# ChaitIITB/ReplicatingGPT

Hardware: AMD Instinct MI355X
Metric: train tokens/sec at 1/2/4/8 MI355X + MFMA util, char-GPT block 256 (higher is better)
Workload: dtype bf16; 1 GPU; c2: char-GPT 6L/6H/384d, block 256, batch 64/GPU, dropout 0.2, AdamW, full train step; global_batch=64, seq_len=256, parallelism=dp1, world_size=1, graph=True

## Files before the change

### include/charpt.h

```cpp
#ifndef CHARPT_H
#define CHARPT_H
#include <stdint.h>

#ifdef __cplusplus
extern "C" {
#endif

enum { CG_OK = 0, CG_EINVAL = 1, CG_EHIP = 2, CG_EUNSUPPORTED = 3 };
enum { CG_F32 = 0, CG_BF16 = 1 };
enum { CG_BITS = 2 };

enum {
    CG_EPI_STORE = 0,
    CG_EPI_BIAS = 1,
    CG_EPI_BIAS_RELU = 2,
    CG_EPI_BIAS_RESID = 3,
    CG_EPI_BIAS_DROP_RESID = 4,
    CG_EPI_RELU_BWD = 5,
    CG_EPI_STORE_ROWDOT = 7
};

typedef struct {
    int kind;
    const float* bias;
    const float* resid;
    int64_t ld_resid;
    const void* aux;
    int aux_dtype;
    int64_t ld_aux;
    double dropout_p;
    uint64_t seed;
    const uint64_t* rng_call;
    int site;
    float beta;
    float* colpart;
    int flags;
} cg_epilogue_t;

enum { CG_GEMM_SLAB_BF16 = 1, CG_GEMM_DEFER_REDUCE = 2 };
enum { CG_DEFER = 1 };

const char* cg_last_error_string(void);
int cg_version(void);
int cg_set_tuning(const char* key, int value);
int64_t cg_gemm_ws_launches(void);
int cg_device_info(int* n_cu, int* arch_major, int* arch_minor);
int cg_timing_event_create(void** event);
int cg_timing_event_record(void* event, void* stream);
int cg_timing_event_elapsed(void* start, void* end, float* ms);
int cg_timing_event_destroy(void* event);

int cg_counter_add(int64_t* counter, int64_t delta, void* stream);
int cg_rng_snapshot(uint64_t* counter, uint64_t* snap, void* stream);
int cg_dropout_mask(float* dst, int64_t n, double p, uint64_t seed, const uint64_t* rng_call, int site,
                    void* stream);
int cg_dropout_apply(const float* x, int64_t rows, int64_t C, int64_t ldx, void* y, int y_dtype, double p,
                     uint64_t seed, const uint64_t* rng_call, int site, void* stream);
int cg_sum_f32(const float* x, int64_t n, float scale, float* out, float* ws, void* stream);
int cg_cast_f32_bf16(const float* x, uint16_t* y, int64_t n, void* stream);

int cg_gather_batch(const void* data, int data_is_u8, const int64_t* ix, int64_t* x, int64_t* y,
                    int64_t B, int64_t T, void* stream);

int cg_gather_pairs(const int64_t* table, const int64_t* plen, const int64_t* tlen, const int64_t* ix, int64_t* x,
                    int64_t* y, int64_t B, int64_t T, int64_t pad_token, int64_t ignore_index, void* stream);

int cg_embed_fwd(const int64_t* idx, const float* wte, const float* wpe, float* x, int64_t B, int64_t T,
                 int64_t C, int64_t V, void* stream);
int64_t cg_embed_bwd_workspace(int64_t B, int64_t T, int64_t C, int64_t V);
int cg_embed_bwd(const int64_t* idx, const float* dx, float* dwte, float* dwpe, int64_t B, int64_t T,
                 int64_t C, int64_t V, int accumulate, void* workspace, void* stream);

int cg_layernorm_fwd(const float* x, const float* w, const float* b, void* y, int y_dtype, float* mean,
                     float* rstd, int64_t rows, int64_t C, float eps, void* stream);
int64_t cg_layernorm_bwd_workspace(int64_t rows, int64_t C);
int cg_layernorm_bwd(const void* dy, int dy_dtype, const float* x, const float* w, const float* mean,
                     const float* rstd, const float* dres, float* dx, uint16_t* dx_bf16, float* dw, float* db,
                     int accumulate, void* workspace, int64_t rows, int64_t C, void* stream);
int cg_layernorm_bwd_ex(const void* dy, int dy_dtype, const float* x, const float* w, const float* mean,
                        const float* rstd, const float* dres, float* dx, uint16_t* lp_out, double lp_dropout_p,
                        uint64_t lp_seed, const uint64_t* lp_rng_call, int lp_site, float* dw, float* db,
                        float* lp_colsum, int accumulate, int colsum_accumulate, void* workspace, int64_t rows,
                        int64_t C, void* stream);
int cg_layernorm_bwd_rows(const void* dy, int dy_dtype, const float* x, const float* w, const float* mean,
                          const float* rstd, const float* dres, float* dx, uint16_t* lp_out, double lp_dropout_p,
                          uint64_t lp_seed, const uint64_t* lp_rng_call, int lp_site, int lp_colsum,
                          void* workspace, int64_t rows, int64_t C, void* stream);
int cg_layernorm_bwd_reduce(const void* workspace, int64_t rows, int64_t C, int lp_colsum_partials, float* dw,
                            float* db, float* lp_colsum, int accumulate, int colsum_accumulate, void* stream);
int cg_layernorm_bwd_reduce_ex(const void* workspace, int64_t rows, int64_t C, int lp_colsum_partials, float* dw,
                               float* db, float* lp_colsum, int accumulate, int colsum_accumulate, int flags,
                               void* stream);

int64_t cg_gemm_workspace(int64_t M, int64_t N, int split_k);
int cg_gemm_colpart_supported(int a_trans, int b_trans, int64_t M, int64_t N, int64_t K, int64_t lda, int64_t ldb,
                              int64_t ldc);
int cg_gemm_relu_bits_supported(int a_trans, int b_trans, int64_t M, int64_t N, int64_t K, int64_t lda, int64_t ldb,
                                int64_t ldc);
// ... 145 lines not shown
```

### replicatinggpt_amd/_lib.py

```python
import ctypes
import os
import re

import torch

_HERE = os.path.dirname(os.path.abspath(__file__))
LIB_PATH = os.environ.get("CHARPT_LIB") or os.path.join(_HERE, "libcharpt_hip.so")
HEADER_PATH = os.path.join(os.path.dirname(_HERE), "include", "charpt.h")

CG_F32, CG_BF16, CG_BITS = 0, 1, 2
EPI_STORE, EPI_BIAS, EPI_BIAS_RELU, EPI_BIAS_RESID, EPI_BIAS_DROP_RESID, EPI_RELU_BWD = range(6)
EPI_STORE_ROWDOT = 7
GEMM_SLAB_BF16, GEMM_DEFER_REDUCE = 1, 2
DEFER = 1

c_i64, c_int, c_dbl, c_flt, c_u64, P = ctypes.c_int64, ctypes.c_int, ctypes.c_double, ctypes.c_float, ctypes.c_uint64, ctypes.c_void_p


class Epilogue(ctypes.Structure):
    _fields_ = [("kind", c_int), ("bias", P), ("resid", P), ("ld_resid", c_i64), ("aux", P), ("aux_dtype", c_int),
                ("ld_aux", c_i64), ("dropout_p", c_dbl), ("seed", c_u64), ("rng_call", P), ("site", c_int),
                ("beta", c_flt), ("colpart", P), ("flags", c_int)]


class WgradProblem(ctypes.Structure):
    _fields_ = [("M", c_i64), ("N", c_i64), ("K", c_i64), ("A", P), ("lda", c_i64), ("B", P), ("ldb", c_i64), ("C", P),
                ("ldc", c_i64), ("beta", c_flt), ("split_k", c_int), ("workspace", P), ("flags", c_int)]


_SIGS = {
    "cg_last_error_string": (ctypes.c_char_p, []),
    "cg_version": (c_int, []),
    "cg_set_tuning": (c_int, [ctypes.c_char_p, c_int]),
    "cg_device_info": (c_int, [P, P, P]),
    "cg_counter_add": (c_int, [P, c_i64, P]),
    "cg_rng_snapshot": (c_int, [P, P, P]),
    "cg_dropout_mask": (c_int, [P, c_i64, c_dbl, c_u64, P, c_int, P]),
    "cg_dropout_apply": (c_int, [P, c_i64, c_i64, c_i64, P, c_int, c_dbl, c_u64, P, c_int, P]),
    "cg_sum_f32": (c_int, [P, c_i64, c_flt, P, P, P]),
    "cg_cast_f32_bf16": (c_int, [P, P, c_i64, P]),
    "cg_gather_batch": (c_int, [P, c_int, P, P, P, c_i64, c_i64, P]),
    "cg_gather_pairs": (c_int, [P, P, P, P, P, P, c_i64, c_i64, c_i64, c_i64, P]),
    "cg_embed_fwd": (c_int, [P, P, P, P, c_i64, c_i64, c_i64, c_i64, P]),
    "cg_embed_bwd_workspace": (c_i64, [c_i64, c_i64, c_i64, c_i64]),
    "cg_embed_bwd": (c_int, [P, P, P, P, c_i64, c_i64, c_i64, c_i64, c_int, P, P]),
    "cg_layernorm_fwd": (c_int, [P, P, P, P, c_int, P, P, c_i64, c_i64, c_flt, P]),
    "cg_layernorm_bwd_workspace": (c_i64, [c_i64, c_i64]),
    "cg_layernorm_bwd": (c_int, [P, c_int, P, P, P, P, P, P, P, P, P, c_int, P, c_i64, c_i64, P]),
    "cg_layernorm_bwd_ex": (c_int, [P, c_int, P, P, P, P, P, P, P, c_dbl, c_u64, P, c_int, P, P, P, c_int, c_int, P,
                                    c_i64, c_i64, P]),
    "cg_layernorm_bwd_rows": (c_int, [P, c_int, P, P, P, P, P, P, P, c_dbl, c_u64, P, c_int, c_int, P, c_i64, c_i64,
                                      P]),
    "cg_layernorm_bwd_reduce": (c_int, [P, c_i64, c_i64, c_int, P, P, P, c_int, c_int, P]),
    "cg_layernorm_bwd_reduce_ex": (c_int, [P, c_i64, c_i64, c_int, P, P, P, c_int, c_int, c_int, P]),
    "cg_gemm_workspace": (c_i64, [c_i64, c_i64, c_int]),
    "cg_gemm_colpart_supported": (c_int, [c_int, c_int, c_i64, c_i64, c_i64, c_i64, c_i64, c_i64]),
    "cg_gemm_relu_bits_supported": (c_int, [c_int, c_int, c_i64, c_i64, c_i64, c_i64, c_i64, c_i64]),
    "cg_gemm_ws_launches": (c_i64, []),
    "cg_gemm_rowdot_supported": (c_int, [c_int, c_int, c_i64, c_i64, c_i64, c_i64, c_i64, c_i64]),
    "cg_linear_rows_f32_supported": (c_int, [c_i64, c_i64, c_i64]),
    "cg_decode_qkv_f32": (c_int, [c_i64, c_i64, c_i64, P, c_i64, P, P, c_flt, P, c_i64, P, c_i64, P, c_i64, P, P, P]),
    "cg_linear_rows_f32": (c_int, [c_i64, c_i64, c_i64, P, c_i64, P, P, c_flt, P, c_i64, P, c_int, P, c_i64, P, c_i64, P]),
    "cg_ffn_fwd_f32_supported": (c_int, [c_i64, c_i64, c_i64]),
    "cg_ffn_fwd_f32": (c_int, [c_i64, c_i64, c_i64, P, c_i64, P, P, c_flt, P, c_i64, P, P, c_i64, P, P, c_i64, P,
                               c_i64, P]),
    "cg_gemm_resid_layernorm_supported": (c_int, [c_i64, c_i64, c_i64]),
    "cg_gemm_resid_layernorm": (c_int, [c_i64, c_i64, c_i64, P, c_i64, P, c_i64, P, c_i64, ctypes.POINTER(Epilogue), P, P,
                                        P, P, P, c_flt, P]),
    "cg_flush_deferred": (c_int, [P]),
    "cg_discard_deferred": (c_int, [P, P]),
    "cg_reduce_rows": (c_int, [P, c_i64, c_i64, P, c_int, P]),
    "cg_reduce_rows_ex": (c_int, [P, c_i64, c_i64, P, c_int, c_int, P]),
    "cg_gemm": (c_int, [c_int, c_int, c_int, c_i64, c_i64, c_i64, P, c_i64, P, c_i64, P, c_int, c_i64,
                        ctypes.POINTER(Epilogue), c_int, P, P]),
    "cg_gemm_wgrad_group_supported": (c_int, [ctypes.POINTER(WgradProblem), c_int]),
    "cg_gemm_wgrad_group": (c_int, [ctypes.POINTER(WgradProblem), c_int, P]),
    "cg_colsum_workspace": (c_i64, [c_i64, c_i64]),
    "cg_colsum": (c_int, [P, c_int, c_i64, c_i64, c_i64, P, c_int, P, P]),
    "cg_attn_fwd": (c_int, [c_int, c_i64, c_i64, c_i64, c_i64, P, P, P, c_i64, P, c_i64, P, c_flt, c_dbl, c_u64, P,
                            c_int, P, P]),
    "cg_attn_fwd_premasked": (c_int, [c_int, c_i64, c_i64, c_i64, c_i64, P, P, P, c_i64, P, c_i64, P, c_flt, c_dbl,
                                      c_u64, P, c_int, P, P]),
    "cg_attn_dropmask": (c_int, [c_i64, c_i64, c_i64, c_dbl, c_u64, P, c_int, P, P]),
    "cg_layernorm_fwd_attn_dropmask": (c_int, [P, P, P, P, c_int, P, P, c_i64, c_i64, c_flt, c_i64, c_i64, c_i64,
                                               c_dbl, c_u64, P, c_int, P, P]),
    "cg_attn_mask_bytes": (c_i64, [c_i64, c_i64, c_i64]),
    "cg_attn_bwd_workspace": (c_i64, [c_i64, c_i64, c_i64, c_i64]),
    "cg_attn_bwd": (c_int, [c_int, c_i64, c_i64, c_i64, c_i64, P, P, P, c_i64, P, c_i64, P, c_i64, P, P, P, P, c_i64,
                            c_flt, c_dbl, c_u64, P, c_int, P, P, P]),
    "cg_attn_bwd_delta": (c_int, [c_int, c_i64, c_i64, c_i64, c_i64, P, P, P, c_i64, P, c_i64, P, c_i64, P, P, P, P,
                                  P, c_i64, c_flt, c_dbl, c_u64, P, c_int, P, P, P]),
    "cg_ce_fwd": (c_int, [P, c_i64, c_i64, c_i64, P, P, P, P]),
    "cg_ce_bwd": (c_int, [P, c_i64, c_i64, c_i64, P, P, P, c_flt, P, c_i64, P, P]),
    "cg_head_workspace": (c_i64, [c_i64, c_i64]),
    "cg_head_fwd": (c_int, [P, P, c_i64, P, P, P, P, P, P, c_i64, c_i64, c_i64, P]),
    "cg_head_bwd": (c_int, [P, P, P, P, c_flt, P, P, c_i64, P, c_int, P, c_i64, c_i64, P]),
    "cg_head_bwd_ex": (c_int, [P, P, P, P, c_flt, P, P, c_i64, P, c_int, P, c_i64, c_i64, c_int, P]),
    "cg_head_masked_workspace": (c_i64, [c_i64, c_i64]),
    "cg_head_fwd_masked": (c_int, [P, P, c_i64, P, P, c_i64, P, P, P, P, P, c_i64, c_i64, c_i64, P]),
    "cg_head_bwd_masked": (c_int, [P, P, P, c_i64, P, P, P, P, c_i64, P, c_int, P, c_i64, c_i64, c_int, P]),
    "cg_ce_fwd_masked": (c_int, [P, c_i64, c_i64, P, c_i64, P, P, P]),
    "cg_ce_mean_masked_workspace": (c_i64, [c_i64]),
    "cg_ce_mean_masked": (c_int, [P, P, c_i64, c_i64, P, P, P, P]),
    "cg_ce_bwd_masked": (c_int, [P, c_i64, c_i64, P, c_i64, P, P, P, P, P, P]),
    "cg_decode_window": (c_int, [P, c_i64, c_i64, c_i64, P, P, P]),
    "cg_decode_embed": (c_int, [P, c_i64, P, P, c_i64, P, P, c_i64, P]),
    "cg_decode_kv_append": (c_int, [P, c_i64, c_i64, c_i64, c_i64, c_i64, c_i64, c_i64, P, P, P, P]),
    "cg_decode_attn": (c_int, [P, c_i64, P, P, c_i64, c_i64, c_i64, c_i64, c_i64, c_i64, P, c_i64, c_flt, P, c_i64,
                               P]),
    "cg_decode_sample": (c_int, [P, c_i64, c_i64, c_i64, c_int, P, P, P, c_i64, P]),
    "cg_decode_sample_filtered": (c_int, [P, c_i64, c_i64, c_i64, P, P, P, P, c_i64, P]),
# ... 71 lines not shown
```

### replicatinggpt_amd/csrc/gemm.hip

```cpp
#include "defer.h"

using namespace cg;

namespace {

constexpr int GBM = 64, GBN = 64, GBK = 16;

template <typename TA, typename TB, typename TC>
__global__ __launch_bounds__(256) void k_gemm_generic(int a_trans, int b_trans, int64_t M, int64_t N, int64_t K,
                                                      const TA* __restrict__ A, int64_t lda,
                                                      const TB* __restrict__ B, int64_t ldb, TC* __restrict__ C,
                                                      int64_t ldc, EpiArgs epi, int split_k, int64_t kchunk,
                                                      float* __restrict__ ws) {
    __shared__ float As[GBK][GBM + 4];
    __shared__ float Bs[GBK][GBN + 4];
    const int tid = threadIdx.x, lane = tid & 63, wave = tid >> 6;
    const int wm = wave >> 1, wn = wave & 1;
    const int64_t tilesN = (N + GBN - 1) / GBN;
    const int64_t m0 = (int64_t)(blockIdx.x / tilesN) * GBM;
    const int64_t n0 = (int64_t)(blockIdx.x % tilesN) * GBN;
    const int split = blockIdx.y;
    const int64_t kb = split * kchunk;
    const int64_t ke = kb + kchunk < K ? kb + kchunk : K;

// ... 80 lines not shown
    a.aux_dtype = e->aux_dtype;
    a.ld_aux = e->ld_aux;
    a.thr = e->dropout_p > 0 ? dropout_threshold(e->dropout_p) : 0u;
    a.dscale = e->dropout_p > 0 ? dropout_scale(e->dropout_p) : 1.f;
    a.seed = e->seed;
    a.rng_call = e->rng_call;
    a.site = e->site;
    a.beta = e->beta;
    a.colpart = e->colpart;
    return a;
}

template <typename TA, typename TB>
int launch_generic(int a_trans, int b_trans, int64_t M, int64_t N, int64_t K, const void* A, int64_t lda,
                   const void* B, int64_t ldb, void* C, int c_dtype, int64_t ldc, const EpiArgs& e, int split_k,
                   void* ws, hipStream_t st) {
    int64_t kchunk = (K + split_k - 1) / split_k;
    kchunk = (kchunk + GBK - 1) / GBK * GBK;
    const int64_t tiles = ((M + GBM - 1) / GBM) * ((N + GBN - 1) / GBN);
    dim3 grid((unsigned)tiles, (unsigned)split_k);
    if (c_dtype == CG_BF16)
        k_gemm_generic<TA, TB, bf16_t><<<grid, 256, 0, st>>>(a_trans, b_trans, M, N, K, (const TA*)A, lda,
                                                             (const TB*)B, ldb, (bf16_t*)C, ldc, e, split_k, kchunk,
                                                             (float*)ws);
    else
        k_gemm_generic<TA, TB, float><<<grid, 256, 0, st>>>(a_trans, b_trans, M, N, K, (const TA*)A, lda,
                                                            (const TB*)B, ldb, (float*)C, ldc, e, split_k, kchunk,
                                                            (float*)ws);
    return CG_OK;
}

}

namespace cg {
int g_gemm_variant = 0;
int g_gemm_max_grid = 0;
int g_gemm_group_p8 = 0;
int g_gemm_group_pk = 0;
int g_gemm_n96 = 1;
}

extern "C" int cg_gemm_colpart_supported(int a_trans, int b_trans, int64_t M, int64_t N, int64_t K, int64_t lda,
                                         int64_t ldb, int64_t ldc) {
    return gemm_colpart_supported(a_trans, b_trans, M, N, K, lda, ldb, ldc) ? 1 : 0;
}

extern "C" int cg_gemm_relu_bits_supported(int a_trans, int b_trans, int64_t M, int64_t N, int64_t K, int64_t lda,
                                           int64_t ldb, int64_t ldc) {
    return gemm_relu_bits_supported(a_trans, b_trans, M, N, K, lda, ldb, ldc) ? 1 : 0;
}

extern "C" int64_t cg_gemm_ws_launches(void) { return (int64_t)ws_gemm_launches(); }

extern "C" int cg_gemm_rowdot_supported(int a_trans, int b_trans, int64_t M, int64_t N, int64_t K, int64_t lda,
                                        int64_t ldb, int64_t ldc) {
    return gemm_rowdot_supported(a_trans, b_trans, M, N, K, lda, ldb, ldc) ? 1 : 0;
}

extern "C" int64_t cg_gemm_workspace(int64_t M, int64_t N, int split_k) {
    return split_k > 1 ? (int64_t)split_k * M * N * (int64_t)sizeof(float) : 0;
}

extern "C" int cg_gemm_resid_layernorm_supported(int64_t M, int64_t N, int64_t K) {
    return gemm_resid_ln_supported(M, N, K) ? 1 : 0;
}

extern "C" int cg_gemm_resid_layernorm(int64_t M, int64_t N, int64_t K, const void* A, int64_t lda, const void* W,
                                       int64_t ldw, float* out, int64_t ldc, const cg_epilogue_t* epi,
                                       const float* ln_w, const float* ln_b, void* y, float* mean, float* rstd,
                                       float eps, void* stream) {
    CG_REQUIRE(gemm_resid_ln_supported(M, N, K),
               "cg_gemm_resid_layernorm: unsupported shape M=%lld N=%lld K=%lld (N == 384, M %% 64 == 0, K %% 64 == 0)",
               (long long)M, (long long)N, (long long)K);
    CG_REQUIRE(epi && (epi->kind == CG_EPI_BIAS_RESID || epi->kind == CG_EPI_BIAS_DROP_RESID) && epi->bias &&
                   epi->resid && epi->beta == 0.f && epi->flags == 0 && !epi->colpart,
               "cg_gemm_resid_layernorm: needs a BIAS_RESID / BIAS_DROP_RESID epilogue with bias and residual, beta 0");
    CG_REQUIRE(A && W && out && ln_w && ln_b && y && mean && rstd, "cg_gemm_resid_layernorm: null pointer");
    CG_REQUIRE(lda >= K && ldw >= K && lda % 8 == 0 && ldw % 8 == 0 && ldc >= N && ldc % 4 == 0 &&
                   epi->ld_resid >= N && epi->ld_resid % 4 == 0,
               "cg_gemm_resid_layernorm: bad leading dimensions");
    CG_REQUIRE((((uintptr_t)A | (uintptr_t)W | (uintptr_t)out | (uintptr_t)epi->resid | (uintptr_t)epi->bias |
                 (uintptr_t)ln_w | (uintptr_t)ln_b | (uintptr_t)y) & 15) == 0,
               "cg_gemm_resid_layernorm: operands must be 16-B aligned");
    const EpiArgs e = make_epi(epi);
    gemm_resid_ln_launch(M, K, (const bf16_t*)A, lda, (const bf16_t*)W, ldw, out, ldc, e, ln_w, ln_b, (bf16_t*)y, mean,
                         rstd, eps, (hipStream_t)stream);
    CG_LAUNCH_CHECK("cg_gemm_resid_layernorm");
    return CG_OK;
}

extern "C" int cg_gemm(int op_dtype, int a_trans, int b_trans, int64_t M, int64_t N, int64_t K, const void* A,
                       int64_t lda, const void* B, int64_t ldb, void* C, int c_dtype, int64_t ldc,
                       const cg_epilogue_t* epi, int split_k, void* workspace, void* stream) {
    CG_REQUIRE(M > 0 && N > 0 && K > 0, "cg_gemm: empty problem M=%lld N=%lld K=%lld", (long long)M, (long long)N,
               (long long)K);
    CG_REQUIRE(split_k >= 1 && split_k <= 64, "cg_gemm: split_k out of range");
    CG_REQUIRE(split_k == 1 || workspace, "cg_gemm: split_k > 1 needs a workspace");
    CG_REQUIRE(op_dtype == CG_BF16 || op_dtype == CG_F32, "cg_gemm: bad op dtype");
    hipStream_t st = (hipStream_t)stream;
    EpiArgs e = make_epi(epi);
    CG_REQUIRE(split_k == 1 || e.kind == CG_EPI_STORE || e.kind == CG_EPI_BIAS || e.kind == CG_EPI_BIAS_RESID,
               "cg_gemm: split-K supports STORE/BIAS/BIAS_RESID epilogues only");
    const bool vec4 = N % 4 == 0 && ldc % 4 == 0 && M * N < (int64_t)1 << 31 &&
                      (((uintptr_t)C | (uintptr_t)workspace | (uintptr_t)(e.bias ? e.bias : (const float*)C) |
                        (uintptr_t)(e.resid ? e.resid : (const float*)C)) & 15) == 0 &&
                      (!e.resid || e.ld_resid % 4 == 0);
// ... 131 lines not shown
```

### replicatinggpt_amd/csrc/gemm_common.h

```cpp
#pragma once
#include <type_traits>

#include "adamw.h"
#include "common.h"

namespace cg {

typedef float fv16f __attribute__((ext_vector_type(16)));

struct EpiArgs {
    int kind;
    const float* bias;
    const float* resid;
    int64_t ld_resid;
    const void* aux;
    int aux_dtype;
    int64_t ld_aux;
    uint32_t thr;
    float dscale;
    uint64_t seed;
    const uint64_t* rng_call;
    int site;
    float beta;
    float* colpart;
// ... 205 lines not shown
        }
        return;
    }
#endif
    for (int q = 0; q < r.na; ++q) {
        const AdamJob& J = r.a[q];
        const AdamScalars sc = adam_scalars(J.lr, J.beta1, J.beta2, J.eps, J.wd, J.step);
        for (int64_t i = t0; i < J.n4; i += nthr) {
            fv4 pv = *(const fv4*)(J.p + 4 * i);
            const fv4 gv = *(const fv4*)(J.g + 4 * i);
            fv4 mv = *(const fv4*)(J.m + 4 * i), vv = *(const fv4*)(J.v + 4 * i);
#pragma unroll
            for (int e = 0; e < 4; ++e) {
                float me = mv[e], ve = vv[e];
                pv[e] = adam_one(pv[e], gv[e], me, ve, sc);
                mv[e] = me;
                vv[e] = ve;
            }
            *(fv4*)(J.p + 4 * i) = pv;
            *(fv4*)(J.m + 4 * i) = mv;
            *(fv4*)(J.v + 4 * i) = vv;
            *(uint2*)(J.pb + 4 * i) = make_uint2(pack_bf2(pv[0], pv[1]), pack_bf2(pv[2], pv[3]));
        }
    }
}

extern int g_gemm_variant;
extern int g_gemm_max_grid;
extern int g_gemm_group_p8;
extern int g_gemm_group_pk;
extern int g_gemm_n96;
extern int g_linear_rows_nb;
extern int g_pk_flags;
int gemm_cu_count();

bool fast_gemm_launch(int at, int bt, int64_t M, int64_t N, int64_t K, const bf16_t* A, int64_t lda, const bf16_t* B,
                      int64_t ldb, void* C, int c_dtype, int64_t ldc, const EpiArgs& e, int split_k, float* ws,
                      hipStream_t st);
bool gemm_colpart_supported(int at, int bt, int64_t M, int64_t N, int64_t K, int64_t lda, int64_t ldb, int64_t ldc);
bool gemm_rowdot_supported(int at, int bt, int64_t M, int64_t N, int64_t K, int64_t lda, int64_t ldb, int64_t ldc);
bool gemm_relu_bits_supported(int at, int bt, int64_t M, int64_t N, int64_t K, int64_t lda, int64_t ldb, int64_t ldc);
bool glds_gemm_launch(int variant, int at, int bt, int64_t M, int64_t N, int64_t K, const bf16_t* A, int64_t lda,
                      const bf16_t* B, int64_t ldb, void* C, int c_dtype, int64_t ldc, const EpiArgs& e, int split_k,
                      float* ws, hipStream_t st);
bool pk_gemm_launch(int variant, int at, int bt, int64_t M, int64_t N, int64_t K, const bf16_t* A, int64_t lda,
                    const bf16_t* B, int64_t ldb, void* C, int c_dtype, int64_t ldc, const EpiArgs& e, int split_k,
                    float* ws, hipStream_t st);

extern int g_gemm_ws;
bool ws_gemm_auto(int64_t M, int64_t N, int kind);
bool ws_gemm_launch(int at, int bt, int64_t M, int64_t N, int64_t K, const bf16_t* A, int64_t lda, const bf16_t* B,
                    int64_t ldb, void* C, int c_dtype, int64_t ldc, const EpiArgs& e, int split_k, hipStream_t st);
long long ws_gemm_launches();

constexpr int MAX_GROUP = 4;
struct GroupProb {
    const bf16_t* A;
    const bf16_t* B;
    void* ws;
    int64_t lda, ldb;
    int M, N;
    int tilesN, ntiles;
    int nkt, nkc;
    int split_k;
    int item0;
    int gm;
};
bool gemm_wgrad_group_ok(int64_t M, int64_t N, int64_t K, const void* A, int64_t lda, const void* B, int64_t ldb,
                         const void* C, int64_t ldc, int split_k);
void pk_group_launch(const GroupProb* probs, int n, bool slab_bf16, hipStream_t st);

bool gemm_resid_ln_supported(int64_t M, int64_t N, int64_t K);
void gemm_resid_ln_launch(int64_t M, int64_t K, const bf16_t* A, int64_t lda, const bf16_t* W, int64_t ldw, float* X,
                          int64_t ldx, const EpiArgs& e, const float* lnw, const float* lnb, bf16_t* Y, float* mean,
                          float* rstd, float eps, hipStream_t st);
bool p8_gemm_launch(int variant, int at, int bt, int64_t M, int64_t N, int64_t K, const bf16_t* A, int64_t lda,
                    const bf16_t* B, int64_t ldb, void* C, int c_dtype, int64_t ldc, const EpiArgs& e, int split_k,
                    float* ws, hipStream_t st);

}
```

### replicatinggpt_amd/csrc/gemm_ws.hip

```cpp
#include "gemm_pk.h"

namespace cg {
int g_gemm_ws = 1;
namespace {
using namespace gt;

long long g_ws_launches = 0;

constexpr int WS_NBUF = 3;
constexpr int WS_KT_A = 64 * 64 * 2;
constexpr int WS_KT_B = 64 * 128 * 2;
constexpr int WS_XCHG = 8 * 1024;
constexpr int WS_BITS = 1024;
constexpr int WS_LPT = 1;
constexpr int WS_STORES = 2;

constexpr int ws_lds_bytes(int nkt) { return WS_NBUF * nkt * WS_KT_A + WS_XCHG + WS_NBUF * WS_BITS; }

__device__ __forceinline__ void store_pair(uint32_t x0, uint32_t y0, uint32_t x1, uint32_t y1, bf16_t* C, int64_t ldc,
                                           int64_t m, int64_t nb, int q) {
    const int64_t col = nb + ((q & 1) ? 16 : 0) + ((q >> 1) ? 8 : 0);
    const auto sx = __builtin_amdgcn_permlane16_swap(x0, x1, false, false);
    const auto sy = __builtin_amdgcn_permlane16_swap(y0, y1, false, false);
    st_out16((uint4*)(C + m * ldc + col), make_uint4(sx[0], sy[0], sx[1], sy[1]));
}

__device__ __forceinline__ float bf_lo(uint32_t w) { return __uint_as_float(w << 16); }
__device__ __forceinline__ float bf_hi(uint32_t w) { return __uint_as_float(w & 0xffff0000u); }

template <bool BT, int EK, int NKT>
__global__ __launch_bounds__(512, 1) __attribute__((amdgpu_waves_per_eu(1, 2)))
void k_gemm_ws(int M, int N, const bf16_t* __restrict__ A, int64_t lda, const bf16_t* __restrict__ B, int64_t ldb,
               bf16_t* __restrict__ C, int64_t ldc, const float* __restrict__ bias, uint32_t* __restrict__ bits,
               int64_t ldw, float* __restrict__ colpart) {
    static_assert(NKT >= 1 && NKT <= 6, "K <= 384");
    constexpr int STAGE = NKT * WS_KT_A;
    static_assert(!BT || NKT * WS_KT_B <= (WS_NBUF - 1) * STAGE, "the transposed panel fits in stages 1..");
    extern __shared__ __attribute__((aligned(16))) char smem[];
    const int tid = threadIdx.x, lane = tid & 63, wave = __builtin_amdgcn_readfirstlane(tid >> 6);
    const int wr = wave >> 2, wc = wave & 3, g = lane >> 4;
    const int npanels = N / 128, P = gridDim.x, bpp = P / npanels;
    const int lb = xcd_remap(blockIdx.x, P);
    const int panel = lb % npanels, rslot = lb / npanels;
    if (rslot >= bpp) return;
    const int T = M / 64, base = T / bpp, rem = T % bpp;
    const int ntile = base + (rslot < rem ? 1 : 0);
    if (ntile == 0) return;
    const int tile0 = rslot * base + (rslot < rem ? rslot : rem);
    const int64_t n0 = (int64_t)panel * 128, nb = n0 + wc * 32;

    const uint32_t lds0 = lds_base(smem);
    char* const xchg = smem + WS_NBUF * STAGE;
    const uint32_t bits0 = lds0 + (uint32_t)(WS_NBUF * STAGE + WS_XCHG);
    DmaP<false, 64, 8, FBK> da;
    da.init(lda, wave, lane);
    auto issue_a = [&](int t, int kt, int sg) {
        const bf16_t* src = A + (int64_t)(tile0 + t) * 64 * lda + kt * FBK;
        da.issue1(src, 0, lds0 + (uint32_t)(sg * STAGE + kt * WS_KT_A), wave);
    };
    const uint32_t bits_off = (uint32_t)(lane * (int)ldw * 4);
    auto issue_bits = [&](int t, int sg) {
        if (EK == CG_EPI_RELU_BWD && wave == 0)
            dma16sl(bits + (int64_t)(tile0 + t) * 64 * ldw + panel * 4, bits_off, bits0 + (uint32_t)(sg * WS_BITS));
    };

    issue_bits(0, 0);
#pragma unroll
    for (int kt = 0; kt < NKT; ++kt) issue_a(0, kt, 0);
    sv8 bw[NKT][2][2];
    if constexpr (!BT) {
#pragma unroll
        for (int kt = 0; kt < NKT; ++kt)
#pragma unroll
            for (int s = 0; s < 2; ++s)
#pragma unroll
                for (int j = 0; j < 2; ++j)
                    bw[kt][s][j] = *(const sv8*)(B + (nb + 16 * j + (lane & 15)) * ldb + kt * FBK + 32 * s + 8 * g);
    } else {
        DmaP<true, 128, 8, FBK> db;
        db.init(ldb, wave, lane);
#pragma unroll
        for (int kt = 0; kt < NKT; ++kt)
#pragma unroll
            for (int i = 0; i < 2; ++i)
                db.issue1(B + (int64_t)kt * FBK * ldb + n0, i, lds0 + (uint32_t)(STAGE + kt * WS_KT_B), wave);
        wait_vm<0>();
        __builtin_amdgcn_s_barrier();
#pragma unroll
        for (int kt = 0; kt < NKT; ++kt)
#pragma unroll
            for (int s = 0; s < 2; ++s)
#pragma unroll
                for (int j = 0; j < 2; ++j)
                    bw[kt][s][j] = frag<true, 128>(smem + STAGE + kt * WS_KT_B, wc * 32 + 16 * j, s, lane);
        asm volatile("s_waitcnt lgkmcnt(0)" ::: "memory");
        __builtin_amdgcn_s_barrier();
    }
    float4 bv[2];
    if constexpr (EK == CG_EPI_BIAS_RELU) {
#pragma unroll
        for (int j = 0; j < 2; ++j) bv[j] = *(const float4*)(bias + nb + 4 * g + 16 * j);
    }
    if (ntile > 1) {
        issue_bits(1, 1);
#pragma unroll
        for (int kt = 0; kt < NKT; ++kt) issue_a(1, kt, 1);
    }

    constexpr int LPT = NKT * WS_LPT;
    int sg = 0;
    for (int t = 0; t < ntile; ++t) {
        const bool more = t + 1 < ntile;
        if (t > 0) {
            if (more) wait_vm<LPT + WS_STORES>();
            else wait_vm<WS_STORES>();
        } else {
            if (more) wait_vm<LPT>();
            else wait_vm<0>();
        }
        asm volatile("s_waitcnt lgkmcnt(0)" ::: "memory");
        __builtin_amdgcn_s_barrier();
        const bool pf = t + 2 < ntile;
        const int sg2 = sg == 0 ? 2 : sg - 1;
        const char* img = smem + sg * STAGE;
        if (pf) issue_bits(t + 2, sg2);

        fv4 acc[2][2];
#pragma unroll
        for (int i = 0; i < 2; ++i)
#pragma unroll
            for (int j = 0; j < 2; ++j) acc[i][j] = fv4{0.f, 0.f, 0.f, 0.f};
        sv8 af[2][2][2];
        auto read_a = [&](int kt) {
#pragma unroll
            for (int s = 0; s < 2; ++s)
#pragma unroll
                for (int i = 0; i < 2; ++i)
                    af[kt & 1][s][i] = frag<false, 64>(img + kt * WS_KT_A, wr * 32 + 16 * i, s, lane);
        };
        read_a(0);
#pragma unroll
        for (int kt = 0; kt < NKT; ++kt) {
            if (kt + 1 < NKT) read_a(kt + 1);
#pragma unroll
            for (int s = 0; s < 2; ++s)
#pragma unroll
                for (int i = 0; i < 2; ++i)
#pragma unroll
                    for (int j = 0; j < 2; ++j) acc[i][j] = mfma_bf16(bw[kt][s][j], af[kt & 1][s][i], acc[i][j]);
            if (pf) issue_a(t + 2, kt, sg2);
        }

        const int64_t mr = (int64_t)(tile0 + t) * 64 + wr * 32 + (lane & 15);
        uint32_t px[2][2], py[2][2];
        if constexpr (EK == CG_EPI_BIAS_RELU) {
            uint32_t w[2];
#pragma unroll
            for (int i = 0; i < 2; ++i) {
#pragma unroll
                for (int j = 0; j < 2; ++j) {
                    fv4& v = acc[i][j];
                    v[0] = fmaxf(v[0] + bv[j].x, 0.f); v[1] = fmaxf(v[1] + bv[j].y, 0.f);
                    v[2] = fmaxf(v[2] + bv[j].z, 0.f); v[3] = fmaxf(v[3] + bv[j].w, 0.f);
                    px[i][j] = pack_bf2(v[0], v[1]);
                    py[i][j] = pack_bf2(v[2], v[3]);
                }
                w[i] = (nz4_bf16(make_uint2(px[i][0], py[i][0])) << (4 * g)) |
                       (nz4_bf16(make_uint2(px[i][1], py[i][1])) << (16 + 4 * g));
                w[i] |= (uint32_t)__shfl_xor((int)w[i], 16, 64);
                w[i] |= (uint32_t)__shfl_xor((int)w[i], 32, 64);
            }
            if (bits && g < 2) bits[(mr + 16 * g) * ldw + (nb >> 5)] = g ? w[1] : w[0];
        } else if constexpr (EK == CG_EPI_RELU_BWD) {
            const char* bimg = smem + WS_NBUF * STAGE + WS_XCHG + sg * WS_BITS;
#pragma unroll
            for (int i = 0; i < 2; ++i) {
                const uint32_t w = *(const uint32_t*)(bimg + (wr * 32 + 16 * i + (lane & 15)) * 16 + wc * 4);
#pragma unroll
                for (int j = 0; j < 2; ++j) {
                    const uint32_t kb = (w >> (16 * j + 4 * g)) & 0xfu;
                    fv4& v = acc[i][j];
#pragma unroll
                    for (int q = 0; q < 4; ++q) v[q] = ((kb >> q) & 1u) ? v[q] : 0.f;
                    px[i][j] = pack_bf2(v[0], v[1]);
                    py[i][j] = pack_bf2(v[2], v[3]);
                }
            }
            if (colpart) {
                uint4* xp = (uint4*)(xchg + (wc * 64 + lane) * 32);
                if (wr == 1) {
                    xp[0] = make_uint4(px[0][0], py[0][0], px[0][1], py[0][1]);
                    xp[1] = make_uint4(px[1][0], py[1][0], px[1][1], py[1][1]);
                }
                asm volatile("s_waitcnt lgkmcnt(0)" ::: "memory");
                __builtin_amdgcn_s_barrier();
                if (wr == 0) {
                    const uint4 o2 = xp[0], o3 = xp[1];
                    const uint32_t u2[2][2] = {{o2.x, o2.y}, {o2.z, o2.w}}, u3[2][2] = {{o3.x, o3.y}, {o3.z, o3.w}};
                    float* cp = colpart + (int64_t)(tile0 + t) * N + nb + 4 * g;
#pragma unroll
                    for (int j = 0; j < 2; ++j) {
                        fv4 s;
                        s[0] = ((bf_lo(px[0][j]) + bf_lo(px[1][j])) + bf_lo(u2[j][0])) + bf_lo(u3[j][0]);
                        s[1] = ((bf_hi(px[0][j]) + bf_hi(px[1][j])) + bf_hi(u2[j][0])) + bf_hi(u3[j][0]);
                        s[2] = ((bf_lo(py[0][j]) + bf_lo(py[1][j])) + bf_lo(u2[j][1])) + bf_lo(u3[j][1]);
                        s[3] = ((bf_hi(py[0][j]) + bf_hi(py[1][j])) + bf_hi(u2[j][1])) + bf_hi(u3[j][1]);
                        fv4 r;
#pragma unroll
                        for (int q = 0; q < 4; ++q) r[q] = row16_sum_dpp(s[q]);
                        if ((lane & 15) == 0) *(fv4*)(cp + 16 * j) = r;
                    }
                }
                __builtin_amdgcn_sched_barrier(0);
            }
        } else {
#pragma unroll
            for (int i = 0; i < 2; ++i)
#pragma unroll
                for (int j = 0; j < 2; ++j) {
                    px[i][j] = pack_bf2(acc[i][j][0], acc[i][j][1]);
                    py[i][j] = pack_bf2(acc[i][j][2], acc[i][j][3]);
                }
        }
#pragma unroll
        for (int i = 0; i < 2; ++i) store_pair(px[i][0], py[i][0], px[i][1], py[i][1], C, ldc, mr + 16 * i, nb, g);
        sg = sg == WS_NBUF - 1 ? 0 : sg + 1;
    }
    wait_vm<0>();
}

template <bool BT, int EK>
void launch_nkt(int nkt, unsigned grid, int M, int N, const bf16_t* A, int64_t lda, const bf16_t* B, int64_t ldb,
                bf16_t* C, int64_t ldc, const float* bias, uint32_t* bits, int64_t ldw, float* colpart, hipStream_t st) {
#define WS(NKT_)                                                                                                   \
    case NKT_:                                                                                                     \
        k_gemm_ws<BT, EK, NKT_><<<grid, 512, ws_lds_bytes(NKT_), st>>>(M, N, A, lda, B, ldb, C, ldc, bias, bits, ldw, \
                                                                      colpart);                                    \
        break
    switch (nkt) {
        WS(1); WS(2); WS(3); WS(4); WS(5); WS(6);
        default: break;
    }
#undef WS
}

}

long long ws_gemm_launches() { return g_ws_launches; }

bool ws_gemm_auto(int64_t M, int64_t N, int kind) {
    const int only = g_gemm_ws == 2 ? CG_EPI_STORE : g_gemm_ws == 3 ? CG_EPI_BIAS_RELU : g_gemm_ws == 4 ? CG_EPI_RELU_BWD : -1;
    return g_gemm_ws && (only < 0 || kind == only) && N >= 1152 && M >= 4096;
}

bool ws_gemm_launch(int at, int bt, int64_t M, int64_t N, int64_t K, const bf16_t* A, int64_t lda, const bf16_t* B,
                    int64_t ldb, void* C, int c_dtype, int64_t ldc, const EpiArgs& e, int split_k, hipStream_t st) {
    if (at || split_k != 1 || e.beta != 0.f || c_dtype != CG_BF16 || g_pk_flags) return false;
    if (K % FBK || K > 6 * FBK || M % 64 || N % 128 || lda % 8 || ldb % 8 || ldc % 8) return false;
    if (M >= ((int64_t)1 << 31) || N >= ((int64_t)1 << 31)) return false;
    if (lda >= ((int64_t)1 << 24) || ldb >= ((int64_t)1 << 24)) return false;
    if ((((uintptr_t)A) | ((uintptr_t)B) | ((uintptr_t)C)) & 15) return false;
    const bool with_bits = e.aux_dtype == CG_BITS && e.aux;
    uint32_t* bits = with_bits ? (uint32_t*)e.aux : nullptr;
    switch (e.kind) {
        case CG_EPI_STORE:
            if (e.colpart) return false;
            break;
        case CG_EPI_BIAS_RELU:
            if (!e.bias || (((uintptr_t)e.bias) & 15) || e.colpart) return false;
            if (e.aux_dtype == CG_BITS && (!e.aux || (((uintptr_t)e.aux) & 3) || e.ld_aux < N / 32)) return false;
            break;
        case CG_EPI_RELU_BWD:
            if (!with_bits || (((uintptr_t)e.aux) & 15) || e.ld_aux % 4 || e.ld_aux < N / 32 ||
                e.ld_aux >= ((int64_t)1 << 24))
                return false;
            if (e.colpart && (((uintptr_t)e.colpart) & 15)) return false;
            break;
        default: return false;
    }
    int64_t P = gemm_cu_count();
    if (g_gemm_max_grid > 0 && g_gemm_max_grid < P) P = g_gemm_max_grid;
    if (P < N / 128) return false;
    const int nkt = (int)(K / FBK);
#define WSL(BT_, EK_)                                                                                               \
    launch_nkt<BT_, EK_>(nkt, (unsigned)P, (int)M, (int)N, A, lda, B, ldb, (bf16_t*)C, ldc, e.bias, bits, e.ld_aux, \
                         e.colpart, st)
    if (e.kind == CG_EPI_STORE) {
        if (bt) WSL(true, CG_EPI_STORE);
        else WSL(false, CG_EPI_STORE);
    } else if (e.kind == CG_EPI_BIAS_RELU) {
        if (bt) WSL(true, CG_EPI_BIAS_RELU);
        else WSL(false, CG_EPI_BIAS_RELU);
    } else {
        if (bt) WSL(true, CG_EPI_RELU_BWD);
        else WSL(false, CG_EPI_RELU_BWD);
    }
#undef WSL
    ++g_ws_launches;
    return true;
}

}
```

Before: 6.071 million tokens/s.

## Split persistent GEMM into 256-thread half-height blocks, two per CU

The persistent bf16 GEMM kernel moves from one 512-thread block per CU (64-row tiles, 8 waves) to 256-thread blocks with 32-row tiles and 4 waves, launching two blocks per CU. The LDS layout is recomputed so the transposed B panel is staged in chunks of up to three k-tiles, and the colpart reduction now accumulates across pairs of tiles in registers instead of through an LDS exchange and barrier. Relu-bits loads are fetched once per 64-row pair of tiles. The aim is to let two independent blocks overlap each other's barriers and loads, at the cost of more B-fragment reloads per CU and a higher per-block LDS floor. Optional timestamp instrumentation and an occupancy query are also added.

```diff
diff --git a/include/charpt.h b/include/charpt.h
--- a/include/charpt.h
+++ b/include/charpt.h
@@ -44,6 +44,7 @@
 int cg_version(void);
 int cg_set_tuning(const char* key, int value);
 int64_t cg_gemm_ws_launches(void);
+int cg_gemm_ws_blocks_per_cu(int b_trans, int kind, int nkt);
 int cg_device_info(int* n_cu, int* arch_major, int* arch_minor);
 int cg_timing_event_create(void** event);
 int cg_timing_event_record(void* event, void* stream);
diff --git a/replicatinggpt_amd/_lib.py b/replicatinggpt_amd/_lib.py
--- a/replicatinggpt_amd/_lib.py
+++ b/replicatinggpt_amd/_lib.py
@@ -57,6 +57,7 @@
     "cg_gemm_colpart_supported": (c_int, [c_int, c_int, c_i64, c_i64, c_i64, c_i64, c_i64, c_i64]),
     "cg_gemm_relu_bits_supported": (c_int, [c_int, c_int, c_i64, c_i64, c_i64, c_i64, c_i64, c_i64]),
     "cg_gemm_ws_launches": (c_i64, []),
+    "cg_gemm_ws_blocks_per_cu": (c_int, [c_int, c_int, c_int]),
     "cg_gemm_rowdot_supported": (c_int, [c_int, c_int, c_i64, c_i64, c_i64, c_i64, c_i64, c_i64]),
     "cg_linear_rows_f32_supported": (c_int, [c_i64, c_i64, c_i64]),
     "cg_decode_qkv_f32": (c_int, [c_i64, c_i64, c_i64, P, c_i64, P, P, c_flt, P, c_i64, P, c_i64, P, c_i64, P, P, P]),
diff --git a/replicatinggpt_amd/csrc/gemm.hip b/replicatinggpt_amd/csrc/gemm.hip
--- a/replicatinggpt_amd/csrc/gemm.hip
+++ b/replicatinggpt_amd/csrc/gemm.hip
@@ -156,6 +156,8 @@
 
 extern "C" int64_t cg_gemm_ws_launches(void) { return (int64_t)ws_gemm_launches(); }
 
+extern "C" int cg_gemm_ws_blocks_per_cu(int b_trans, int kind, int nkt) { return ws_gemm_blocks_per_cu(b_trans, kind, nkt); }
+
 extern "C" int cg_gemm_rowdot_supported(int a_trans, int b_trans, int64_t M, int64_t N, int64_t K, int64_t lda,
                                         int64_t ldb, int64_t ldc) {
     return gemm_rowdot_supported(a_trans, b_trans, M, N, K, lda, ldb, ldc) ? 1 : 0;
diff --git a/replicatinggpt_amd/csrc/gemm_common.h b/replicatinggpt_amd/csrc/gemm_common.h
--- a/replicatinggpt_amd/csrc/gemm_common.h
+++ b/replicatinggpt_amd/csrc/gemm_common.h
@@ -281,6 +281,7 @@
 bool ws_gemm_launch(int at, int bt, int64_t M, int64_t N, int64_t K, const bf16_t* A, int64_t lda, const bf16_t* B,
                     int64_t ldb, void* C, int c_dtype, int64_t ldc, const EpiArgs& e, int split_k, hipStream_t st);
 long long ws_gemm_launches();
+int ws_gemm_blocks_per_cu(int bt, int kind, int nkt);
 
 constexpr int MAX_GROUP = 4;
 struct GroupProb {
diff --git a/replicatinggpt_amd/csrc/gemm_ws.hip b/replicatinggpt_amd/csrc/gemm_ws.hip
--- a/replicatinggpt_amd/csrc/gemm_ws.hip
+++ b/replicatinggpt_amd/csrc/gemm_ws.hip
@@ -8,14 +8,53 @@
 long long g_ws_launches = 0;
 
 constexpr int WS_NBUF = 3;
-constexpr int WS_KT_A = 64 * 64 * 2;
 constexpr int WS_KT_B = 64 * 128 * 2;
-constexpr int WS_XCHG = 8 * 1024;
 constexpr int WS_BITS = 1024;
 constexpr int WS_LPT = 1;
 constexpr int WS_STORES = 2;
 
-constexpr int ws_lds_bytes(int nkt) { return WS_NBUF * nkt * WS_KT_A + WS_XCHG + WS_NBUF * WS_BITS; }
+template <int NKT>
+struct WsGeo {
+    static constexpr int WAVES = 4, ROWS = 32;
+    static constexpr int KT_A = ROWS * 64 * 2;
+    static constexpr int STAGE = NKT * KT_A;
+    static constexpr int PK = NKT < 3 ? NKT : 3;
+    static constexpr int RING = WS_NBUF * STAGE > PK * WS_KT_B ? WS_NBUF * STAGE : PK * WS_KT_B;
+    static constexpr int PANEL = RING - PK * WS_KT_B;
+    static constexpr int NBITS = 2;
+    static constexpr int LDS = RING + NBITS * WS_BITS;
+};
+
+#ifdef CG_WS_STAMPS
+constexpr int WS_ST_TILES = 24, WS_ST_WORDS = 8 + 3 * WS_ST_TILES, WS_ST_BLOCKS = 1024;
+constexpr int WS_ST_LDS = WS_ST_WORDS * 8;
+__device__ unsigned long long g_ws_stamps[WS_ST_BLOCKS * WS_ST_WORDS];
+__device__ __forceinline__ unsigned long long ws_where() {
+    uint32_t hw, xcc;
+    asm volatile("s_getreg_b32 %0, hwreg(HW_REG_HW_ID)" : "=s"(hw));
+    asm volatile("s_getreg_b32 %0, hwreg(HW_REG_XCC_ID)" : "=s"(xcc));
+    return ((unsigned long long)(xcc & 0xff) << 32) | hw;
+}
+#define WS_STAMP_AT(slot, v)                                                  \
+    do {                                                                      \
+        if (threadIdx.x == 0) ((volatile unsigned long long*)stamps)[slot] = (v); \
+    } while (0)
+#define WS_STAMP(slot) WS_STAMP_AT(slot, __builtin_amdgcn_s_memrealtime())
+#define WS_STAMP_TILE(t, k)                                  \
+    do {                                                     \
+        if ((t) < WS_ST_TILES) WS_STAMP(8 + 3 * (t) + (k));  \
+    } while (0)
+#else
+constexpr int WS_ST_LDS = 0;
+#define WS_STAMP_AT(slot, v)
+#define WS_STAMP(slot)
+#define WS_STAMP_TILE(t, k)
+#endif
+
+constexpr int ws_lds_bytes(int nkt) {
+    return nkt == 1 ? WsGeo<1>::LDS : nkt == 2 ? WsGeo<2>::LDS : nkt == 3 ? WsGeo<3>::LDS :
+           nkt == 4 ? WsGeo<4>::LDS : nkt == 5 ? WsGeo<5>::LDS : WsGeo<6>::LDS;
+}
 
 __device__ __forceinline__ void store_pair(uint32_t x0, uint32_t y0, uint32_t x1, uint32_t y1, bf16_t* C, int64_t ldc,
                                            int64_t m, int64_t nb, int q) {
@@ -29,44 +68,55 @@
 __device__ __forceinline__ float bf_hi(uint32_t w) { return __uint_as_float(w & 0xffff0000u); }
 
 template <bool BT, int EK, int NKT>
-__global__ __launch_bounds__(512, 1) __attribute__((amdgpu_waves_per_eu(1, 2)))
+__global__ __launch_bounds__(256, 2) __attribute__((amdgpu_waves_per_eu(1, 2)))
 void k_gemm_ws(int M, int N, const bf16_t* __restrict__ A, int64_t lda, const bf16_t* __restrict__ B, int64_t ldb,
                bf16_t* __restrict__ C, int64_t ldc, const float* __restrict__ bias, uint32_t* __restrict__ bits,
                int64_t ldw, float* __restrict__ colpart) {
     static_assert(NKT >= 1 && NKT <= 6, "K <= 384");
-    constexpr int STAGE = NKT * WS_KT_A;
-    static_assert(!BT || NKT * WS_KT_B <= (WS_NBUF - 1) * STAGE, "the transposed panel fits in stages 1..");
+    using G = WsGeo<NKT>;
+    constexpr int STAGE = G::STAGE, ROWS = G::ROWS;
+    constexpr int UT = EK == CG_EPI_RELU_BWD ? 2 : 1;
     extern __shared__ __attribute__((aligned(16))) char smem[];
     const int tid = threadIdx.x, lane = tid & 63, wave = __builtin_amdgcn_readfirstlane(tid >> 6);
-    const int wr = wave >> 2, wc = wave & 3, g = lane >> 4;
+    const int wc = wave, g = lane >> 4;
     const int npanels = N / 128, P = gridDim.x, bpp = P / npanels;
     const int lb = xcd_remap(blockIdx.x, P);
     const int panel = lb % npanels, rslot = lb / npanels;
     if (rslot >= bpp) return;
-    const int T = M / 64, base = T / bpp, rem = T % bpp;
-    const int ntile = base + (rslot < rem ? 1 : 0);
+    const int T = M / (ROWS * UT), base = T / bpp, rem = T % bpp;
+    const int ntile = (base + (rslot < rem ? 1 : 0)) * UT;
     if (ntile == 0) return;
-    const int tile0 = rslot * base + (rslot < rem ? rslot : rem);
+    const int64_t row0 = (int64_t)(rslot * base + (rslot < rem ? rslot : rem)) * (ROWS * UT);
     const int64_t n0 = (int64_t)panel * 128, nb = n0 + wc * 32;
 
     const uint32_t lds0 = lds_base(smem);
-    char* const xchg = smem + WS_NBUF * STAGE;
-    const uint32_t bits0 = lds0 + (uint32_t)(WS_NBUF * STAGE + WS_XCHG);
-    DmaP<false, 64, 8, FBK> da;
+    const uint32_t bits0 = lds0 + (uint32_t)G::RING;
+#ifdef CG_WS_STAMPS
+    char* const stamps = smem + G::LDS;
+    WS_STAMP(0);
+    WS_STAMP_AT(3, ws_where());
+    WS_STAMP_AT(4, (unsigned long long)ntile);
+    WS_STAMP_AT(5, (unsigned long long)lb);
+#endif
+    DmaP<false, ROWS, G::WAVES, FBK> da;
     da.init(lda, wave, lane);
     auto issue_a = [&](int t, int kt, int sg) {
-        const bf16_t* src = A + (int64_t)(tile0 + t) * 64 * lda + kt * FBK;
-        da.issue1(src, 0, lds0 + (uint32_t)(sg * STAGE + kt * WS_KT_A), wave);
+        const bf16_t* src = A + (row0 + (int64_t)t * ROWS) * lda + kt * FBK;
+        da.issue1(src, 0, lds0 + (uint32_t)(sg * STAGE + kt * G::KT_A), wave);
     };
     const uint32_t bits_off = (uint32_t)(lane * (int)ldw * 4);
-    auto issue_bits = [&](int t, int sg) {
+    auto issue_bits = [&](int u, int slot) {
         if (EK == CG_EPI_RELU_BWD && wave == 0)
-            dma16sl(bits + (int64_t)(tile0 + t) * 64 * ldw + panel * 4, bits_off, bits0 + (uint32_t)(sg * WS_BITS));
+            dma16sl(bits + (row0 + (int64_t)u * 64) * ldw + panel * 4, bits_off, bits0 + (uint32_t)(slot * WS_BITS));
     };
-
-    issue_bits(0, 0);
-#pragma unroll
-    for (int kt = 0; kt < NKT; ++kt) issue_a(0, kt, 0);
+    auto issue_tile0 = [&]() {
+        issue_bits(0, 0);
+#pragma unroll
+        for (int kt = 0; kt < NKT; ++kt) issue_a(0, kt, 0);
+    };
+
+    constexpr bool EARLY0 = !BT || STAGE <= G::PANEL;
+    if constexpr (EARLY0) issue_tile0();
     sv8 bw[NKT][2][2];
     if constexpr (!BT) {
 #pragma unroll
@@ -77,38 +127,44 @@
                 for (int j = 0; j < 2; ++j)
                     bw[kt][s][j] = *(const sv8*)(B + (nb + 16 * j + (lane & 15)) * ldb + kt * FBK + 32 * s + 8 * g);
     } else {
-        DmaP<true, 128, 8, FBK> db;
+        using DB = DmaP<true, 128, G::WAVES, FBK>;
+        DB db;
         db.init(ldb, wave, lane);
 #pragma unroll
-        for (int kt = 0; kt < NKT; ++kt)
-#pragma unroll
-            for (int i = 0; i < 2; ++i)
-                db.issue1(B + (int64_t)kt * FBK * ldb + n0, i, lds0 + (uint32_t)(STAGE + kt * WS_KT_B), wave);
-        wait_vm<0>();
-        __builtin_amdgcn_s_barrier();
-#pragma unroll
-        for (int kt = 0; kt < NKT; ++kt)
-#pragma unroll
-            for (int s = 0; s < 2; ++s)
-#pragma unroll
-                for (int j = 0; j < 2; ++j)
-                    bw[kt][s][j] = frag<true, 128>(smem + STAGE + kt * WS_KT_B, wc * 32 + 16 * j, s, lane);
-        asm volatile("s_waitcnt lgkmcnt(0)" ::: "memory");
-        __builtin_amdgcn_s_barrier();
-    }
+        for (int k0 = 0; k0 < NKT; k0 += G::PK) {
+#pragma unroll
+            for (int kt = k0; kt < k0 + G::PK && kt < NKT; ++kt)
+#pragma unroll
+                for (int i = 0; i < DB::PER_WAVE; ++i)
+                    db.issue1(B + (int64_t)kt * FBK * ldb + n0, i, lds0 + (uint32_t)(G::PANEL + (kt - k0) * WS_KT_B), wave);
+            wait_vm<0>();
+            __builtin_amdgcn_s_barrier();
+#pragma unroll
+            for (int kt = k0; kt < k0 + G::PK && kt < NKT; ++kt)
+#pragma unroll
+                for (int s = 0; s < 2; ++s)
+#pragma unroll
+                    for (int j = 0; j < 2; ++j)
+                        bw[kt][s][j] = frag<true, 128>(smem + G::PANEL + (kt - k0) * WS_KT_B, wc * 32 + 16 * j, s, lane);
+            asm volatile("s_waitcnt lgkmcnt(0)" ::: "memory");
+            __builtin_amdgcn_s_barrier();
+        }
+    }
+    if constexpr (!EARLY0) issue_tile0();
     float4 bv[2];
     if constexpr (EK == CG_EPI_BIAS_RELU) {
 #pragma unroll
         for (int j = 0; j < 2; ++j) bv[j] = *(const float4*)(bias + nb + 4 * g + 16 * j);
     }
     if (ntile > 1) {
-        issue_bits(1, 1);
 #pragma unroll
         for (int kt = 0; kt < NKT; ++kt) issue_a(1, kt, 1);
     }
+    WS_STAMP(1);
 
     constexpr int LPT = NKT * WS_LPT;
     int sg = 0;
+    fv4 slo[2];
     for (int t = 0; t < ntile; ++t) {
         const bool more = t + 1 < ntile;
         if (t > 0) {
@@ -120,10 +176,11 @@
         }
         asm volatile("s_waitcnt lgkmcnt(0)" ::: "memory");
         __builtin_amdgcn_s_barrier();
+        WS_STAMP_TILE(t, 0);
         const bool pf = t + 2 < ntile;
         const int sg2 = sg == 0 ? 2 : sg - 1;
         const char* img = smem + sg * STAGE;
-        if (pf) issue_bits(t + 2, sg2);
+        if (pf && !(t & 1)) issue_bits(t / 2 + 1, (t / 2 + 1) & 1);
 
         fv4 acc[2][2];
 #pragma unroll
@@ -136,7 +193,7 @@
             for (int s = 0; s < 2; ++s)
 #pragma unroll
                 for (int i = 0; i < 2; ++i)
-                    af[kt & 1][s][i] = frag<false, 64>(img + kt * WS_KT_A, wr * 32 + 16 * i, s, lane);
+                    af[kt & 1][s][i] = frag<false, 64>(img + kt * G::KT_A, 16 * i, s, lane);
         };
         read_a(0);
 #pragma unroll
@@ -150,8 +207,9 @@
                     for (int j = 0; j < 2; ++j) acc[i][j] = mfma_bf16(bw[kt][s][j], af[kt & 1][s][i], acc[i][j]);
             if (pf) issue_a(t + 2, kt, sg2);
         }
-
-        const int64_t mr = (int64_t)(tile0 + t) * 64 + wr * 32 + (lane & 15);
+        WS_STAMP_TILE(t, 1);
+
+        const int64_t mr = row0 + (int64_t)t * ROWS + (lane & 15);
         uint32_t px[2][2], py[2][2];
         if constexpr (EK == CG_EPI_BIAS_RELU) {
             uint32_t w[2];
@@ -172,10 +230,10 @@
             }
             if (bits && g < 2) bits[(mr + 16 * g) * ldw + (nb >> 5)] = g ? w[1] : w[0];
         } else if constexpr (EK == CG_EPI_RELU_BWD) {
-            const char* bimg = smem + WS_NBUF * STAGE + WS_XCHG + sg * WS_BITS;
+            const char* bimg = smem + G::RING + ((t >> 1) & 1) * WS_BITS + (t & 1) * 32 * 16;
 #pragma unroll
             for (int i = 0; i < 2; ++i) {
-                const uint32_t w = *(const uint32_t*)(bimg + (wr * 32 + 16 * i + (lane & 15)) * 16 + wc * 4);
+                const uint32_t w = *(const uint32_t*)(bimg + (16 * i + (lane & 15)) * 16 + wc * 4);
 #pragma unroll
                 for (int j = 0; j < 2; ++j) {
                     const uint32_t kb = (w >> (16 * j + 4 * g)) & 0xfu;
@@ -187,24 +245,23 @@
                 }
             }
             if (colpart) {
-                uint4* xp = (uint4*)(xchg + (wc * 64 + lane) * 32);
-                if (wr == 1) {
-                    xp[0] = make_uint4(px[0][0], py[0][0], px[0][1], py[0][1]);
-                    xp[1] = make_uint4(px[1][0], py[1][0], px[1][1], py[1][1]);
-                }
-                asm volatile("s_waitcnt lgkmcnt(0)" ::: "memory");
-                __builtin_amdgcn_s_barrier();
-                if (wr == 0) {
-                    const uint4 o2 = xp[0], o3 = xp[1];
-                    const uint32_t u2[2][2] = {{o2.x, o2.y}, {o2.z, o2.w}}, u3[2][2] = {{o3.x, o3.y}, {o3.z, o3.w}};
-                    float* cp = colpart + (int64_t)(tile0 + t) * N + nb + 4 * g;
+                if (!(t & 1)) {
+#pragma unroll
+                    for (int j = 0; j < 2; ++j) {
+                        slo[j][0] = bf_lo(px[0][j]) + bf_lo(px[1][j]);
+                        slo[j][1] = bf_hi(px[0][j]) + bf_hi(px[1][j]);
+                        slo[j][2] = bf_lo(py[0][j]) + bf_lo(py[1][j]);
+                        slo[j][3] = bf_hi(py[0][j]) + bf_hi(py[1][j]);
+                    }
+                } else {
+                    float* cp = colpart + (row0 / 64 + (t >> 1)) * N + nb + 4 * g;
 #pragma unroll
                     for (int j = 0; j < 2; ++j) {
                         fv4 s;
-                        s[0] = ((bf_lo(px[0][j]) + bf_lo(px[1][j])) + bf_lo(u2[j][0])) + bf_lo(u3[j][0]);
-                        s[1] = ((bf_hi(px[0][j]) + bf_hi(px[1][j])) + bf_hi(u2[j][0])) + bf_hi(u3[j][0]);
-                        s[2] = ((bf_lo(py[0][j]) + bf_lo(py[1][j])) + bf_lo(u2[j][1])) + bf_lo(u3[j][1]);
-                        s[3] = ((bf_hi(py[0][j]) + bf_hi(py[1][j])) + bf_hi(u2[j][1])) + bf_hi(u3[j][1]);
+                        s[0] = (slo[j][0] + bf_lo(px[0][j])) + bf_lo(px[1][j]);
+                        s[1] = (slo[j][1] + bf_hi(px[0][j])) + bf_hi(px[1][j]);
+                        s[2] = (slo[j][2] + bf_lo(py[0][j])) + bf_lo(py[1][j]);
+                        s[3] = (slo[j][3] + bf_hi(py[0][j])) + bf_hi(py[1][j]);
                         fv4 r;
 #pragma unroll
                         for (int q = 0; q < 4; ++q) r[q] = row16_sum_dpp(s[q]);
@@ -224,24 +281,44 @@
         }
 #pragma unroll
         for (int i = 0; i < 2; ++i) store_pair(px[i][0], py[i][0], px[i][1], py[i][1], C, ldc, mr + 16 * i, nb, g);
+        WS_STAMP_TILE(t, 2);
         sg = sg == WS_NBUF - 1 ? 0 : sg + 1;
     }
     wait_vm<0>();
-}
+#ifdef CG_WS_STAMPS
+    WS_STAMP(2);
+    if (tid == 0 && blockIdx.x < WS_ST_BLOCKS) {
+        volatile unsigned long long* out = g_ws_stamps + (size_t)blockIdx.x * WS_ST_WORDS;
+        for (int i = 0; i < WS_ST_WORDS; ++i) out[i] = ((volatile unsigned long long*)stamps)[i];
+    }
+#endif
+}
+
+using ws_fn = void (*)(int, int, const bf16_t*, int64_t, const bf16_t*, int64_t, bf16_t*, int64_t, const float*, uint32_t*,
+                       int64_t, float*);
 
 template <bool BT, int EK>
-void launch_nkt(int nkt, unsigned grid, int M, int N, const bf16_t* A, int64_t lda, const bf16_t* B, int64_t ldb,
-                bf16_t* C, int64_t ldc, const float* bias, uint32_t* bits, int64_t ldw, float* colpart, hipStream_t st) {
-#define WS(NKT_)                                                                                                   \
-    case NKT_:                                                                                                     \
-        k_gemm_ws<BT, EK, NKT_><<<grid, 512, ws_lds_bytes(NKT_), st>>>(M, N, A, lda, B, ldb, C, ldc, bias, bits, ldw, \
-                                                                      colpart);                                    \
-        break
+ws_fn pick_nkt(int nkt) {
     switch (nkt) {
-        WS(1); WS(2); WS(3); WS(4); WS(5); WS(6);
-        default: break;
-    }
-#undef WS
+        case 1: return k_gemm_ws<BT, EK, 1>;
+        case 2: return k_gemm_ws<BT, EK, 2>;
+        case 3: return k_gemm_ws<BT, EK, 3>;
+        case 4: return k_gemm_ws<BT, EK, 4>;
+        case 5: return k_gemm_ws<BT, EK, 5>;
+        case 6: return k_gemm_ws<BT, EK, 6>;
+        default: return nullptr;
+    }
+}
+ws_fn pick(int bt, int kind, int nkt, int& lds) {
+    if (nkt < 1 || nkt > 6) return nullptr;
+    lds = ws_lds_bytes(nkt) + WS_ST_LDS;
+    if (lds < 56 * 1024) lds = 56 * 1024;
+    switch (kind) {
+        case CG_EPI_STORE: return bt ? pick_nkt<true, CG_EPI_STORE>(nkt) : pick_nkt<false, CG_EPI_STORE>(nkt);
+        case CG_EPI_BIAS_RELU: return bt ? pick_nkt<true, CG_EPI_BIAS_RELU>(nkt) : pick_nkt<false, CG_EPI_BIAS_RELU>(nkt);
+        case CG_EPI_RELU_BWD: return bt ? pick_nkt<true, CG_EPI_RELU_BWD>(nkt) : pick_nkt<false, CG_EPI_RELU_BWD>(nkt);
+        default: return nullptr;
+    }
 }
 
 }
@@ -278,26 +355,37 @@
             break;
         default: return false;
     }
-    int64_t P = gemm_cu_count();
+    int64_t P = (int64_t)gemm_cu_count() * 2;
     if (g_gemm_max_grid > 0 && g_gemm_max_grid < P) P = g_gemm_max_grid;
     if (P < N / 128) return false;
-    const int nkt = (int)(K / FBK);
-#define WSL(BT_, EK_)                                                                                               \
-    launch_nkt<BT_, EK_>(nkt, (unsigned)P, (int)M, (int)N, A, lda, B, ldb, (bf16_t*)C, ldc, e.bias, bits, e.ld_aux, \
-                         e.colpart, st)
-    if (e.kind == CG_EPI_STORE) {
-        if (bt) WSL(true, CG_EPI_STORE);
-        else WSL(false, CG_EPI_STORE);
-    } else if (e.kind == CG_EPI_BIAS_RELU) {
-        if (bt) WSL(true, CG_EPI_BIAS_RELU);
-        else WSL(false, CG_EPI_BIAS_RELU);
-    } else {
-        if (bt) WSL(true, CG_EPI_RELU_BWD);
-        else WSL(false, CG_EPI_RELU_BWD);
-    }
-#undef WSL
+    int lds = 0;
+    const ws_fn fn = pick(bt, e.kind, (int)(K / FBK), lds);
+    if (!fn) return false;
+    fn<<<(unsigned)P, 256, lds, st>>>((int)M, (int)N, A, lda, B, ldb, (bf16_t*)C, ldc, e.bias, bits, e.ld_aux,
+                                         e.colpart);
     ++g_ws_launches;
     return true;
 }
 
-}
+int ws_gemm_blocks_per_cu(int bt, int kind, int nkt) {
+    int lds = 0, n = 0;
+    const ws_fn fn = pick(bt, kind, nkt, lds);
+    if (!fn || hipOccupancyMaxActiveBlocksPerMultiprocessor(&n, (const void*)fn, 256, (size_t)lds) != hipSuccess)
+        return -1;
+    return n;
+}
+
+#ifdef CG_WS_STAMPS
+extern "C" int cg_debug_ws_stamps(unsigned long long* host, int nblocks) {
+    if (nblocks < 0 || nblocks > WS_ST_BLOCKS) return 1;
+    return hipMemcpyFromSymbol(host, HIP_SYMBOL(g_ws_stamps), (size_t)nblocks * WS_ST_WORDS * sizeof(unsigned long long)) ==
+                   hipSuccess ? 0 : 1;
+}
+extern "C" int cg_debug_ws_stamps_reset() {
+    static unsigned long long z[WS_ST_BLOCKS * WS_ST_WORDS];
+    return hipMemcpyToSymbol(HIP_SYMBOL(g_ws_stamps), z, sizeof(z)) == hipSuccess ? 0 : 1;
+}
+extern "C" int cg_debug_ws_stamps_words() { return WS_ST_WORDS; }
+#endif
+
+}
```

Measured after the change: 6.154 million tokens/s, median of 6. +1.4%, better.
